# levayz/diffusion_finetuning

Measured on AMD Instinct MI355X. Metric: images/s SD1.5 LoRA rank-4 512^2 train step, higher is better.
Workload: dtype f16; 1 GPU; SD1.5 UNet-only LoRA rank=4, batch=4/GPU, 512^2 (64x64x4 latents), f16 storage/compute, fp32 accumulate + fp32 master LoRA, full train step (fwd+bwd+clip+AdamW); global_batch=4, parallelism=dp1, lora_params=1246464, overflow=False, hipgraph=True, conv_autotune=True, rccl_ranks=1

## Files before the change

### diffusion_finetuning_amd/_native.py

```python
import ctypes
import os
import threading

import torch

_LIB_PATH = os.environ.get("DFA_LIB_PATH") or os.path.join(os.path.dirname(os.path.abspath(__file__)), "lib", "liblora_hip.so")
_lib = None
_lock = threading.Lock()

ABI_VERSION = 9
PROF_KINDS = 18

_DTYPE_CODE = {torch.float32: 0, torch.float16: 1, torch.bfloat16: 2}

_vp, _i64, _i32, _f32 = ctypes.c_void_p, ctypes.c_int64, ctypes.c_int, ctypes.c_float


class GradProblem(ctypes.Structure):
    _fields_ = [
        ("S", _vp), ("P", _vp), ("out", _vp * 4),
        ("s_stride", _i64), ("p_stride", _i64), ("part_stride", _i64), ("M", _i64),
        ("C", _i32), ("r", _i32), ("rg", _i32), ("out_kn", _i32), ("n_blocks", _i32),
        ("scale", _f32),
    ]
# ... 67 lines not shown
                                       ctypes.c_uint64, ctypes.c_uint64, _i32, _i32, _vp]),
    "ddpm_posterior_sample": (_i32, [_vp, _i32, _vp, _vp, _i32, _i64, _f32, _vp]),
    "ddpm_noise_prologue_offset": (_i32, [_vp, _vp, _vp, _vp, _vp, _vp, _vp, _i32, _i64, _i32, ctypes.c_uint64, ctypes.c_uint64,
                                          _i32, _i32, _i64, _f32, _vp, _vp]),
    "ddpm_posterior_prologue_offset": (_i32, [_vp, _i32, _vp, _vp, _vp, _vp, _vp, _vp, _vp, _vp, _i32, _i64, _i32, _f32,
                                              ctypes.c_uint64, ctypes.c_uint64, _i32, _i32, _i64, _f32, _vp, _vp]),
    "ddpm_sample_init": (_i32, [_vp, _vp, _vp, _vp, _vp, _i32, _i64, _i32, _i32, ctypes.c_uint64, _i32, _vp]),
    "ddpm_sample_step": (_i32, [_vp, _vp, _vp, _vp, _vp, _vp, _vp, _vp, _i32, _i64, _i32, _i32, _f32, _i32, _vp]),
    "ddpm_sample_advance": (_i32, [_vp, _i32, _vp]),
    "ddpm_sample_multistep": (_i32, [_vp, _vp, _vp, _vp, _vp, _vp, _vp, _vp, _vp, _vp, _i32, _i64, _i32, _i32, _f32, _i32, _vp]),
    "ddpm_sample_init_from": (_i32, [_vp, _vp, _vp, _vp, _vp, _vp, _vp, _i32, _i64, _i32, _i32, _f32, _f32, _i32, ctypes.c_uint64,
                                     _i32, _vp]),
    "ddpm_sample_step_keep": (_i32, [_vp] * 11 + [_i32, _i64, _i64, _i32, _i32, _f32, _i32, _vp]),
    "ddpm_sample_multistep_keep": (_i32, [_vp] * 13 + [_i32, _i64, _i64, _i32, _i32, _f32, _i32, _vp]),
    "ddpm_sample_init_shared": (_i32, [_vp, _vp, _vp, _vp, _vp, _i32, _i64, _i32, _i32, ctypes.c_uint64, _i32, _vp]),
    "ddpm_sample_step_shared": (_i32, [_vp, _vp, _vp, _vp, _vp, _vp, _vp, _vp, _i32, _i64, _i32, _i32, _f32, _i32, _vp]),
    "ddpm_sample_init_from_shared": (_i32, [_vp, _vp, _vp, _vp, _vp, _vp, _vp, _i32, _i64, _i32, _i32, _f32, _f32, _i32,
                                            ctypes.c_uint64, _i32, _vp]),
    "ddpm_sample_step_keep_shared": (_i32, [_vp] * 11 + [_i32, _i64, _i64, _i32, _i32, _f32, _i32, _vp]),
    "ddpm_sample_multistep_keep_shared": (_i32, [_vp] * 13 + [_i32, _i64, _i64, _i32, _i32, _f32, _i32, _vp]),
    "ddpm_sample_sigma_init": (_i32, [_vp] * 7 + [_i32, _i64, _i32, _i32, _f32, _f32, _f32, _i32, _i32, ctypes.c_uint64, _i32, _vp]),
    "ddpm_sample_sigma": (_i32, [_vp] * 14 + [_i32, _i64, _i64, _i32, _i32, _i32, _f32, _i32, _vp]),
    "ddpm_cfg_rescale": (_i32, [_vp, _vp, _i32, _i64, _f32, _f32, _i32, _vp]),
    "embed_rows_fwd": (_i32, [_vp, _vp, _vp, _i64, _i32, _i64, _i32, _vp]),
    "embed_rows_bwd": (_i32, [_vp, _vp, _vp, _vp, _i64, _i32, _i64, _i32, _i32, _vp]),
    "lora_adamw_rows": (_i32, [_vp, _vp, _vp, _vp, _vp, _i64, _i32, _vp, _f32, _f32, _f32, _f32, _f32, _f32, _f32, _i32, _vp]),
    "ti_rows_grad": (_i32, [_vp, _vp, _i64, _i32, _vp, _i32, _vp, _i32, _i32, _vp]),
    "ti_rows_adamw_decay": (_i32, [_vp, _i64, _i32, _vp, _i32, _vp, _vp, _vp, _f32, _f32, _f32, _f32, _f32, _f32, _i32, _f32, _f32,
                                   _vp]),
    "geglu_linear_bwd": (_i32, [_vp, _vp, _vp, _vp, _vp, _i64, _i32, _i32, _i32, _vp]),
    "geglu_gate_fwd": (_i32, [_vp, _vp, _i64, _i32, _i32, _vp]),
    "geglu_gate_bwd": (_i32, [_vp, _vp, _vp, _i64, _i32, _i32, _vp]),
    "attn_split_heads": (_i32, [_vp, _vp, _i32, _i32, _i32, _i32, _i32, _i32, _vp]),
    "attn_merge_heads": (_i32, [_vp, _vp, _i32, _i32, _i32, _i32, _i32, _i32, _vp]),
    "attn_merge_heads_strided": (_i32, [_vp, _vp, _i32, _i32, _i32, _i32, _i32, _i64, _i64, _i64, _i32, _vp]),
    "group_norm_act_workspace_bytes": (_i64, [_i32, _i32, _i32, _i32, _i32, _i32]),
    "group_norm_act_plan": (_i32, [_i32, _i32, _i32, _i32, _i32, _i32]),
    "group_norm_act_fwd": (_i32, [_vp] * 8 + [_i32, _i32, _i32, _i32, _f32, _i32, _i32, _i32, _vp]),
    "group_norm_act_bwd": (_i32, [_vp] * 10 + [_i32, _i32, _i32, _i32, _i32, _i32, _i32, _vp]),
    "group_norm_act_bwd_res": (_i32, [_vp] * 11 + [_i32, _i32, _i32, _i32, _i32, _i32, _vp]),
    "residual_bias_add_supported": (_i32, [_i32, _i32, _i32, _i32]),
    "residual_bias_add": (_i32, [_vp] * 5 + [_i32, _i32, _i32, _i32, _vp]),
    "tokens_nchw_supported": (_i32, [_i32, _i32, _i32, _i32]),
    "tokens_to_nchw_add": (_i32, [_vp] * 3 + [_i32, _i32, _i32, _i32, _vp]),
    "nchw_to_tokens": (_i32, [_vp] * 2 + [_i32, _i32, _i32, _i32, _vp]),
    "time_proj_supported": (_i32, [_i32, _i32, _i32]),
    "time_proj_all": (_i32, [_vp] * 6 + [_i32, _i32, _i32, _i32, _vp]),
    "conv3x3_small_supported": (_i32, [_i32, _i32, _i32, _i32, _i32, _i32]),
    "conv3x3_small_workspace_bytes": (_i64, [_i32, _i32, _i32, _i32, _i32, _i32]),
    "conv3x3_small_plan": (_i32, [_i64, _i32, _i32, _i32]),
    "conv3x3_small_plan_channels": (_i32, [_i32, _i32, _i32]),
    "conv3x3_small_pack": (_i32, [_vp, _vp, _i32, _i32, _i32, _i32, _vp]),
    "conv3x3_small": (_i32, [_vp] * 5 + [_i64, _i32, _i32, _i32, _i32, _i32, _i32, _vp]),
    "conv3x3_large_supported": (_i32, [_i32, _i32, _i32, _i32, _i32, _i32]),
    "conv3x3_large_workspace_bytes": (_i64, [_i32, _i32, _i32, _i32, _i32, _i32]),
    "conv3x3_large_plan": (_i32, [_i64, _i32, _i32, _i32]),
    "conv3x3_large_plan_channels": (_i32, [_i32, _i32, _i32]),
    "conv3x3_large": (_i32, [_vp] * 5 + [_i64, _i32, _i32, _i32, _i32, _i32, _i32, _vp]),
    "conv3x3_large_tile_choice": (_i32, [_i32, _i32, _i32, _i32, _i32, _i32]),
    "conv3x3_large_tile": (_i32, [_vp] * 5 + [_i64, _i32, _i32, _i32, _i32, _i32, _i32, _i32, _vp]),
    "add_layer_norm_max_channels": (_i32, []),
    "add_layer_norm_fwd": (_i32, [_vp] * 8 + [_i64, _i32, _f32, _i32, _vp]),
    "add_layer_norm_bwd": (_i32, [_vp] * 7 + [_i64, _i32, _i32, _vp]),
    "attn_ctx_supported": (_i32, [_i32, _i32, _i32, _i32, _i32, _i32]),
    "attn_ctx_fwd": (_i32, [_vp, _vp, _vp, _vp, _i32, _i32, _i32, _i32, _i32, _f32, _i32, _vp]),
    "attn_ctx_bwd_workspace_bytes": (_i64, [_i32, _i32, _i32, _i32, _i32]),
    "attn_ctx_fwd_strided": (_i32, [_vp, _vp, _vp, _vp, _i64, _i32, _i32, _i32, _i32, _i32, _f32, _i32, _vp]),
    "attn_ctx_bwd_strided": (_i32, [_vp] * 8 + [_i64, _i64, _i32, _i32, _i32, _i32, _i32, _f32, _i32, _vp]),
    "attn_flash_fwd_strided": (_i32, [_vp, _vp, _vp, _vp, _vp, _i64, _i32, _i32, _i32, _i32, _i32, _f32, _i32, _vp]),
    "attn_flash_bwd_strided": (_i32, [_vp] * 10 + [_i64, _i64, _i32, _i32, _i32, _i32, _i32, _f32, _i32, _vp]),
    "attn_ctx_bwd": (_i32, [_vp, _vp, _vp, _vp, _vp, _vp, _vp, _vp, _i32, _i32, _i32, _i32, _i32, _f32, _i32, _vp]),
    "attn_causal_supported": (_i32, [_i32, _i32, _i32, _i32, _i32]),
    "attn_causal_fwd_strided": (_i32, [_vp, _vp, _vp, _vp, _i64, _i32, _i32, _i32, _i32, _f32, _i32, _vp]),
    "attn_causal_bwd_workspace_bytes": (_i64, [_i32, _i32, _i32, _i32]),
    "attn_causal_bwd_strided": (_i32, [_vp] * 8 + [_i64, _i64, _i32, _i32, _i32, _i32, _f32, _i32, _vp]),
    "attn_flash_supported": (_i32, [_i32, _i32, _i32, _i32, _i32, _i32]),
    "attn_flash_fwd": (_i32, [_vp, _vp, _vp, _vp, _vp, _i32, _i32, _i32, _i32, _i32, _f32, _i32, _vp]),
    "attn_flash_bwd_workspace_bytes": (_i64, [_i32, _i32, _i32]),
    "attn_flash_bwd": (_i32, [_vp] * 10 + [_i32, _i32, _i32, _i32, _i32, _f32, _i32, _vp]),
    "attn_f32_supported": (_i32, [_i32, _i32, _i32, _i32, _i32]),
    "attn_f32_fwd": (_i32, [_vp, _vp, _vp, _vp, _vp, _i32, _i32, _i32, _i32, _i32, _f32, _vp]),
    "attn_f32_bwd_workspace_bytes": (_i64, [_i32, _i32, _i32]),
    "attn_f32_bwd": (_i32, [_vp] * 10 + [_i32, _i32, _i32, _i32, _i32, _f32, _vp]),
    "lora_distill_workspace_bytes": (_i64, [_i64, _i64]),
    "lora_distill_start": (_i32, [_vp, _i32, _i64, _i32, _i64, _vp, _vp]),
    "lora_distill_diff": (_i32, [_vp, _i32, _i64, _i32, _i32, _vp, _vp]),
    "lora_distill_rayleigh_ritz": (_i32, [_vp, _i32, _i32, _i32, ctypes.c_double, _i32, _vp, _vp]),
    "lora_distill_finalize": (_i32, [_vp, _i32, _i32, _f32, _i32, _vp, _vp, _vp]),
    "lora_quantile_clamp": (_i32, [_vp, _i64, _f32, _vp, _vp]),
    "lora_distill_wide_width": (_i32, [_i32]),
    "lora_distill_wide_workspace_bytes": (_i64, [_i64, _i64, _i32]),
    "lora_distill_wide_start": (_i32, [_vp, _i32, _i64, _i32, _i64, _vp, _vp]),
    "lora_distill_wide_diff": (_i32, [_vp, _i32, _i64, _i32, _i32, _i32, _vp, _vp]),
    "lora_distill_wide_rayleigh_ritz": (_i32, [_vp, _i32, _i32, _i32, ctypes.c_double, _i32, _vp, _vp]),
    "lora_distill_wide_finalize": (_i32, [_vp, _i32, _i32, _f32, _i32, _vp, _vp, _vp]),
    "lora_prof_enable": (_i32, [_i32]),
    "lora_prof_collect": (_i32, [ctypes.POINTER(ProfTotals)]),
    "lora_prof_null_mode": (_i32, [_i32]),
    "lora_prof_kernel_name": (ctypes.c_char_p, [_i32]),
}


def library_path() -> str:
    return _LIB_PATH


def lib():
# ... 1210 lines not shown
def time_proj_supported(N: int, E: int, dtype) -> bool:
    return dtype in (torch.float16, torch.bfloat16) and bool(lib().time_proj_supported(N, E, dtype_code(dtype)))


def time_proj_all(temb, weights, biases, extra_biases):
    _require_device(temb, *weights)
    N, E = temb.shape
    L = len(weights)
    widths = [w.shape[0] for w in weights]
    out = torch.empty(N * sum(widths), dtype=temb.dtype, device=temb.device)
    ptrs = lambda ts: (_vp * L)(*[None if t is None else t.data_ptr() for t in ts])
    _check(lib().time_proj_all(_ptr(temb), ptrs(weights), ptrs(biases), ptrs(extra_biases), (_i32 * L)(*widths), _ptr(out), L, N, E,
                               dtype_code(temb.dtype), _stream(temb)), "time_proj_all")
    outs, off = [], 0
    for c in widths:
        outs.append(out[off:off + N * c].view(N, c))
        off += N * c
    return outs


def conv3x3_small_supported(N: int, Cin: int, Cout: int, H: int, W: int, dtype) -> bool:
    return dtype in (torch.float16, torch.bfloat16) and bool(lib().conv3x3_small_supported(N, Cin, Cout, H, W, dtype_code(dtype)))


def conv3x3_small_plan(pixels: int, Cin: int, Cout: int, dtype) -> bool:
    return dtype in (torch.float16, torch.bfloat16) and bool(lib().conv3x3_small_plan(int(pixels), Cin, Cout, dtype_code(dtype)))


def conv3x3_small_plan_channels(Cin: int, Cout: int, dtype) -> bool:
    return dtype in (torch.float16, torch.bfloat16) and bool(lib().conv3x3_small_plan_channels(Cin, Cout, dtype_code(dtype)))


def conv3x3_small_pack(weight, backward: bool):
    _require_device(weight)
    Cout, Cin = weight.shape[:2]
    packed = torch.empty(weight.numel(), dtype=weight.dtype, device=weight.device)
    _check(lib().conv3x3_small_pack(_ptr(weight), _ptr(packed), Cin, Cout, int(backward), dtype_code(weight.dtype),
                                    _stream(weight)), "conv3x3_small_pack")
    return packed


def conv3x3_small(x, pack, bias, Cout: int):
    _require_device(x, pack, bias)
    N, Cin, H, W = x.shape
    code = dtype_code(x.dtype)
    nbytes = int(lib().conv3x3_small_workspace_bytes(N, Cin, Cout, H, W, code))
    ws = torch.empty(max(nbytes, 16) // 4, dtype=torch.float32, device=x.device)
    y = torch.empty((N, Cout, H, W), dtype=x.dtype, device=x.device)
    _check(lib().conv3x3_small(_ptr(x), _ptr(pack), _ptr(bias), _ptr(y), _ptr(ws), nbytes, N, Cin, Cout, H, W, code, _stream(x)),
           "conv3x3_small")
    return y


def conv3x3_large_supported(N: int, Cin: int, Cout: int, H: int, W: int, dtype) -> bool:
    return dtype in (torch.float16, torch.bfloat16) and bool(lib().conv3x3_large_supported(N, Cin, Cout, H, W, dtype_code(dtype)))


def conv3x3_large_plan(pixels: int, Cin: int, Cout: int, dtype) -> bool:
    return dtype in (torch.float16, torch.bfloat16) and bool(lib().conv3x3_large_plan(int(pixels), Cin, Cout, dtype_code(dtype)))


def conv3x3_large_plan_channels(Cin: int, Cout: int, dtype) -> bool:
    return dtype in (torch.float16, torch.bfloat16) and bool(lib().conv3x3_large_plan_channels(Cin, Cout, dtype_code(dtype)))


def conv3x3_large(x, pack, bias, Cout: int):
    _require_device(x, pack, bias)
    N, Cin, H, W = x.shape
    y = torch.empty((N, Cout, H, W), dtype=x.dtype, device=x.device)
    _check(lib().conv3x3_large(_ptr(x), _ptr(pack), _ptr(bias), _ptr(y), None, 0, N, Cin, Cout, H, W, dtype_code(x.dtype),
                               _stream(x)), "conv3x3_large")
    return y


def conv3x3_large_tile_choice(N: int, Cin: int, Cout: int, H: int, W: int, dtype) -> int:
    if dtype not in (torch.float16, torch.bfloat16):
        return -1
    return int(lib().conv3x3_large_tile_choice(N, Cin, Cout, H, W, dtype_code(dtype)))


def conv3x3_large_tile(x, pack, bias, Cout: int, tile: int):
    _require_device(x, pack, bias)
    N, Cin, H, W = x.shape
    y = torch.empty((N, Cout, H, W), dtype=x.dtype, device=x.device)
    _check(lib().conv3x3_large_tile(_ptr(x), _ptr(pack), _ptr(bias), _ptr(y), None, 0, N, Cin, Cout, H, W, dtype_code(x.dtype),
                                    int(tile), _stream(x)), "conv3x3_large_tile")
    return y


def tokens_nchw_supported(N: int, C: int, HW: int, dtype) -> bool:
    return dtype in (torch.float16, torch.bfloat16) and bool(lib().tokens_nchw_supported(N, C, HW, dtype_code(dtype)))


def tokens_to_nchw_add(tok, res, shape):
    _require_device(tok, res)
    N, C, H, W = shape
    out = torch.empty(shape, dtype=tok.dtype, device=tok.device)
    _check(lib().tokens_to_nchw_add(_ptr(tok), _ptr(res), _ptr(out), N, C, H * W, dtype_code(tok.dtype), _stream(tok)),
           "tokens_to_nchw_add")
    return out


def nchw_to_tokens(x):
    _require_device(x)
    N, C, H, W = x.shape
    tok = torch.empty((N, H * W, C), dtype=x.dtype, device=x.device)
# ... 278 lines not shown
```

### diffusion_finetuning_amd/csrc/conv_small.hip

```cpp
#include "conv_common.h"

namespace {

constexpr int kNT = 128;

template <typename T, int MT, int PER>
__global__ __launch_bounds__(kThreads) void conv_small_kernel(const T* __restrict__ x, const T* __restrict__ wp,
                                                              float* __restrict__ part, int Cin, int Cout, int H, int W, int M,
                                                              int mtiles, int ntiles, int cps, int chunks, int Mpad) {
    using Frag = typename Mfma<T>::Frag;
    constexpr int MF = MT / 32;
    extern __shared__ __attribute__((aligned(16))) unsigned char smem[];
    const int tid = threadIdx.x, lane = tid & 63, wave = tid >> 6, wm = wave & 1, wn = wave >> 1;

    int mt, nt, sl;
    {
        const unsigned total = gridDim.x, id = blockIdx.x;
        const unsigned q = total >> 3, rem = total & 7, xcd = id & 7, slot = id >> 3;
        const unsigned n = (xcd < rem ? xcd * (q + 1) : rem * (q + 1) + (xcd - rem) * q) + slot;
        mt = (int)(n % (unsigned)mtiles);
        const unsigned rest = n / (unsigned)mtiles;
        nt = (int)(rest % (unsigned)ntiles);
        sl = (int)(rest / (unsigned)ntiles);
    }
    const int c_begin = sl * cps, c_end = min(c_begin + cps, chunks);
    const int HW = H * W, W2 = W + 2, PP = (H + 2) * W2;
    const int m0 = mt * MT;
    const int q0 = padded_pos(m0, H, W);
    const int P = tile_positions(m0, MT, M, H, W);
    const int qlo = q0 - (W2 + 1);
    const float inv_pp = 1.f / (float)PP, inv_w2 = 1.f / (float)W2;

    int xoff[PER];
    bool in_tile[PER];
#pragma unroll
    for (int s = 0; s < PER; ++s) {
        const int p = tid + s * kThreads;
        const int q = qlo + p, img = fast_div(q, PP, inv_pp), r = q - img * PP, hp = fast_div(r, W2, inv_w2), wq = r - hp * W2;
        in_tile[s] = p < P;
        const bool inside = in_tile[s] && hp >= 1 && hp <= H && wq >= 1 && wq <= W;
        xoff[s] = inside ? img * Cin * HW + (hp - 1) * W + (wq - 1) : -1;
    }
    T raw[PER][32];
    auto load_stage = [&](int cc) {
        const T* base = x + (size_t)cc * kChunk * HW;
#pragma unroll
        for (int s = 0; s < PER; ++s) {
            const int o = xoff[s] >= 0 ? xoff[s] : 0;
#pragma unroll
            for (int c = 0; c < 32; ++c) raw[s][c] = base[o + c * HW];
        }
    };

    int lpos[MF];
    const float inv_hw = 1.f / (float)HW, inv_w = 1.f / (float)W;
#pragma unroll
    for (int f = 0; f < MF; ++f) {
        const int m = min(m0 + wm * (MT / 2) + f * 16 + (lane & 15), M - 1);
        const int img = fast_div(m, HW, inv_hw), r = m - img * HW, h = fast_div(r, W, inv_w);
        lpos[f] = (img * PP + (h + 1) * W2 + (r - h * W) + 1 - q0) * kPitch + (lane >> 4) * 16;
    }
    const int KO = Cout >> 4;
    int wofs[4];
#pragma unroll
    for (int g = 0; g < 4; ++g) wofs[g] = min(nt * (kNT / 16) + wn * 4 + g, KO - 1) * 512 + lane * 8;
    const size_t tap_stride = (size_t)KO * 512;
    const int L_end = c_end * 9;
    Frag wf[9][4];
    auto load_w = [&](int slot, int L) {
        const T* src = wp + (size_t)min(L, L_end - 1) * tap_stride;
#pragma unroll
        for (int g = 0; g < 4; ++g) wf[slot][g] = *reinterpret_cast<const Frag*>(src + wofs[g]);
    };

    f32x4 acc[MF][4];
#pragma unroll
    for (int f = 0; f < MF; ++f)
#pragma unroll
        for (int g = 0; g < 4; ++g) acc[f][g] = f32x4{0.f, 0.f, 0.f, 0.f};

    load_stage(c_begin);
#pragma unroll
    for (int t = 0; t < 9; ++t) load_w(t, c_begin * 9 + t);
    for (int cc = c_begin; cc < c_end; ++cc) {
        __syncthreads();
#pragma unroll
        for (int s = 0; s < PER; ++s)
            if (in_tile[s]) {
#pragma unroll
                for (int c8 = 0; c8 < 4; ++c8) {
                    Frag v;
#pragma unroll
                    for (int j = 0; j < 8; ++j) v[j] = xoff[s] >= 0 ? raw[s][c8 * 8 + j] : static_cast<T>(0.f);
                    *reinterpret_cast<Frag*>(smem + (tid + s * kThreads) * kPitch + c8 * 16) = v;
                }
            }
        __syncthreads();
        load_stage(min(cc + 1, c_end - 1));
        __builtin_amdgcn_sched_barrier(0);
        Frag xf[2][MF];
#pragma unroll
        for (int f = 0; f < MF; ++f) xf[0][f] = *reinterpret_cast<const Frag*>(smem + lpos[f]);
#pragma unroll
        for (int t = 0; t < 9; ++t) {
            if (t + 1 < 9) {
                const int sh = (((t + 1) / 3) * W2 + ((t + 1) % 3)) * kPitch;
#pragma unroll
                for (int f = 0; f < MF; ++f) xf[(t + 1) & 1][f] = *reinterpret_cast<const Frag*>(smem + lpos[f] + sh);
            }
#pragma unroll
            for (int f = 0; f < MF; ++f)
#pragma unroll
                for (int g = 0; g < 4; ++g) acc[f][g] = Mfma<T>::run(xf[t & 1][f], wf[t][g], acc[f][g]);
            load_w(t, cc * 9 + t + 9);
            __builtin_amdgcn_sched_barrier(0);
        }
    }

#pragma unroll
    for (int g = 0; g < 4; ++g) {
        const int k = nt * kNT + wn * 64 + g * 16 + (lane & 15);
        if (k < Cout) {
            float* dst = part + ((size_t)sl * Cout + k) * Mpad + m0 + wm * (MT / 2) + (lane >> 4) * 4;
#pragma unroll
            for (int f = 0; f < MF; ++f) *reinterpret_cast<f32x4*>(dst + f * 16) = acc[f][g];
        }
    }
}

template <typename T, int V>
__global__ __launch_bounds__(256) void conv_small_reduce_kernel(const float* __restrict__ part, const T* __restrict__ bias,
                                                                T* __restrict__ y, int Cout, int HW, int M, int Mpad, int S) {
    const int idx = blockIdx.x * 256 + threadIdx.x, MV = M / V;
    if (idx >= Cout * MV) return;
    const int k = idx / MV, m = (idx - k * MV) * V;
    const float* src = part + (size_t)k * Mpad + m;
    const size_t stride = (size_t)Cout * Mpad;
    float v[V];
    if constexpr (V == 4) {
        f32x4 a = *reinterpret_cast<const f32x4*>(src);
        int s = 1;
        for (; s + 3 < S; s += 4) {
            const f32x4 b0 = *reinterpret_cast<const f32x4*>(src + s * stride), b1 = *reinterpret_cast<const f32x4*>(src + (s + 1) * stride),
                        b2 = *reinterpret_cast<const f32x4*>(src + (s + 2) * stride), b3 = *reinterpret_cast<const f32x4*>(src + (s + 3) * stride);
            a += b0, a += b1, a += b2, a += b3;
        }
        for (; s < S; ++s) a += *reinterpret_cast<const f32x4*>(src + s * stride);
#pragma unroll
        for (int i = 0; i < 4; ++i) v[i] = a[i];
    } else {
        v[0] = src[0];
        for (int s = 1; s < S; ++s) v[0] += src[s * stride];
    }
    const float b = bias ? to_f32(bias[k]) : 0.f;
    const int n = m / HW, p = m - n * HW;
    T* dst = y + ((size_t)n * Cout + k) * HW + p;
    if constexpr (V == 4) {
        struct alignas(8) Out4 { T v[4]; } o;
#pragma unroll
        for (int i = 0; i < 4; ++i) o.v[i] = from_f32<T>(v[i] + b);
        *reinterpret_cast<Out4*>(dst) = o;
    } else {
        dst[0] = from_f32<T>(v[0] + b);
    }
}

template <typename T>
__global__ __launch_bounds__(256) void conv_small_pack_kernel(const T* __restrict__ w, T* __restrict__ out, int Cin, int Cout,
                                                              int backward) {
    const int64_t total = (int64_t)Cin * Cout * 9, o = (int64_t)blockIdx.x * 256 + threadIdx.x;
    if (o >= total) return;
    const int Co = backward ? Cin : Cout, KO = Co >> 4;
    const int j = (int)(o & 7), l = (int)((o >> 3) & 63);
    const int64_t rest = o >> 9;
    const int ko = (int)(rest % KO);
    const int64_t rest2 = rest / KO;
    const int t = (int)(rest2 % 9), cc = (int)(rest2 / 9);
    const int ci = cc * 32 + (l >> 4) * 8 + j, co = ko * 16 + (l & 15);
    const int64_t src = backward ? ((int64_t)ci * Cin + co) * 9 + (8 - t) : ((int64_t)co * Cin + ci) * 9 + t;
    out[o] = w[src];
}

struct Geo {
    int MT = 0, per = 0, mtiles = 0, ntiles = 0, chunks = 0, cps = 0, S = 0, Pcap = 0, Mpad = 0, M = 0;
    int64_t ws_bytes = 0;
    bool ok = false;
};

Geo conv_geo(int N, int Cin, int Cout, int H, int W) {
    Geo g;
    if (!conv_shape_in_range(N, Cin, Cout, H, W)) return g;
    const int M = N * H * W;
    const int mts[2] = {128, 64}, per[2] = {1, 3};
    for (int v = 0; v < 2 && !g.ok; ++v) {
        const int MT = mts[v], mtiles = (M + MT - 1) / MT;
        int pmax = 0;
        for (int t = 0; t < mtiles; ++t) {
            const int p = tile_positions(t * MT, MT, M, H, W);
            pmax = p > pmax ? p : pmax;
        }
        if (pmax > per[v] * kThreads) continue;
        g.MT = MT, g.per = per[v], g.mtiles = mtiles, g.Pcap = pmax, g.ok = true;
    }
    if (!g.ok) return g;
    g.M = M;
    g.Mpad = g.mtiles * g.MT;
    g.ntiles = (Cout + kNT - 1) / kNT;
    g.chunks = Cin / kChunk;
    const int tiles = g.mtiles * g.ntiles, want = kCUs / tiles > 1 ? kCUs / tiles : 1;
    int cps = (g.chunks + want - 1) / want;
    if (g.chunks >= 4 && cps < 2) cps = 2;
    g.cps = cps;
    g.S = (g.chunks + cps - 1) / cps;
    g.ws_bytes = (int64_t)g.S * Cout * g.Mpad * 4;
    if ((int64_t)tiles * g.S > (1 << 20)) g.ok = false;
    return g;
}

template <typename T, int MT, int PER>
bool launch_main(const T* x, const T* wp, float* part, int Cin, int Cout, int H, int W, const Geo& g, hipStream_t s) {
    const int lds = g.Pcap * kPitch;
    auto kern = conv_small_kernel<T, MT, PER>;
    if (lds > 48 * 1024 &&
        hipFuncSetAttribute(reinterpret_cast<const void*>(kern), hipFuncAttributeMaxDynamicSharedMemorySize, lds) != hipSuccess)
        return false;
    hipLaunchKernelGGL(kern, dim3(g.mtiles * g.ntiles * g.S), dim3(kThreads), lds, s, x, wp, part, Cin, Cout, H, W, g.M, g.mtiles,
                       g.ntiles, g.cps, g.chunks, g.Mpad);
    return true;
}

template <typename T>
int run_conv(const void* x_, const void* wp_, const void* bias_, void* y_, void* ws, int Cin, int Cout, int H, int W, const Geo& g,
             hipStream_t s) {
    const T *x = static_cast<const T*>(x_), *wp = static_cast<const T*>(wp_), *bias = static_cast<const T*>(bias_);
    float* part = static_cast<float*>(ws);
    const bool ok = g.MT == 128 ? launch_main<T, 128, 1>(x, wp, part, Cin, Cout, H, W, g, s)
                                : launch_main<T, 64, 3>(x, wp, part, Cin, Cout, H, W, g, s);
    if (!ok) return LORA_E_LAUNCH;
    if ((H * W) % 4 == 0) {
        const int total = Cout * (g.M / 4);
        hipLaunchKernelGGL((conv_small_reduce_kernel<T, 4>), dim3((total + 255) / 256), dim3(256), 0, s, part, bias, static_cast<T*>(y_),
                           Cout, H * W, g.M, g.Mpad, g.S);
    } else {
        const int total = Cout * g.M;
        hipLaunchKernelGGL((conv_small_reduce_kernel<T, 1>), dim3((total + 255) / 256), dim3(256), 0, s, part, bias, static_cast<T*>(y_),
                           Cout, H * W, g.M, g.Mpad, g.S);
    }
    LORA_LAUNCH_CHECK();
    return LORA_OK;
}

}

extern "C" int conv3x3_small_supported(int N, int C_in, int C_out, int H, int W, int dtype) {
    return (dtype == LORA_F16 || dtype == LORA_BF16) && conv_geo(N, C_in, C_out, H, W).ok ? 1 : 0;
}

extern "C" int64_t conv3x3_small_workspace_bytes(int N, int C_in, int C_out, int H, int W, int dtype) {
    if (!conv3x3_small_supported(N, C_in, C_out, H, W, dtype)) return 0;
    return conv_geo(N, C_in, C_out, H, W).ws_bytes;
}

namespace {
bool plan_channels(int C_in, int C_out, int64_t pixels ) {
    if (C_in != 1280 && C_out != 1280) return false;
    const int other = C_in == 1280 ? C_out : C_in;
    const bool at256 = other == 1280 || other == 2560;
    const bool at1024 = other == 640 || other == 1280 || other == 1920 || other == 2560;
    return pixels == 256 ? at256 : pixels == 1024 ? at1024 : pixels == 0 ? (at256 || at1024) : false;
}
}

extern "C" int conv3x3_small_plan(int64_t pixels, int C_in, int C_out, int dtype) {
    if (dtype != LORA_F16 && dtype != LORA_BF16) return 0;
    return pixels >= 1 && plan_channels(C_in, C_out, pixels) ? 1 : 0;
}

extern "C" int conv3x3_small_plan_channels(int C_in, int C_out, int dtype) {
    if (dtype != LORA_F16 && dtype != LORA_BF16) return 0;
    return plan_channels(C_in, C_out, 0) ? 1 : 0;
}

extern "C" int conv3x3_small_pack(const void* w, void* packed, int C_in, int C_out, int backward, int dtype, void* stream) {
    if (!w || !packed || C_in < 1 || C_out < 1 || (backward != 0 && backward != 1)) return LORA_E_BADARG;
    if (dtype != LORA_F16 && dtype != LORA_BF16) return dtype == LORA_F32 ? LORA_E_UNSUPPORTED : LORA_E_BADARG;
    if (C_in % 32 || C_out % 32) return LORA_E_UNSUPPORTED;
    if (!aligned16(packed)) return LORA_E_ALIGN;
    const int64_t total = (int64_t)C_in * C_out * 9;
    if (total >= (1ll << 31)) return LORA_E_UNSUPPORTED;
    hipStream_t s = static_cast<hipStream_t>(stream);
    const dim3 grid((unsigned)((total + 255) / 256));
    if (dtype == LORA_F16)
        hipLaunchKernelGGL(conv_small_pack_kernel<half_t>, grid, dim3(256), 0, s, static_cast<const half_t*>(w),
                           static_cast<half_t*>(packed), C_in, C_out, backward);
    else
        hipLaunchKernelGGL(conv_small_pack_kernel<bf16_t>, grid, dim3(256), 0, s, static_cast<const bf16_t*>(w),
                           static_cast<bf16_t*>(packed), C_in, C_out, backward);
    LORA_LAUNCH_CHECK();
    return LORA_OK;
}

extern "C" int conv3x3_small(const void* x, const void* wpack, const void* bias, void* y, void* workspace, int64_t workspace_bytes,
                             int N, int C_in, int C_out, int H, int W, int dtype, void* stream) {
    if (!x || !wpack || !y || !workspace || N < 1 || C_in < 1 || C_out < 1 || H < 1 || W < 1) return LORA_E_BADARG;
    if (dtype != LORA_F16 && dtype != LORA_BF16) return dtype == LORA_F32 ? LORA_E_UNSUPPORTED : LORA_E_BADARG;
    const Geo g = conv_geo(N, C_in, C_out, H, W);
    if (!g.ok) return LORA_E_UNSUPPORTED;
    if (workspace_bytes < g.ws_bytes) return LORA_E_BADARG;
    if (!aligned16(x) || !aligned16(wpack) || !aligned16(y) || !aligned16(workspace)) return LORA_E_ALIGN;
    hipStream_t s = static_cast<hipStream_t>(stream);
    return dtype == LORA_F16 ? run_conv<half_t>(x, wpack, bias, y, workspace, C_in, C_out, H, W, g, s)
                             : run_conv<bf16_t>(x, wpack, bias, y, workspace, C_in, C_out, H, W, g, s);
}
```

### include/lora_hip.h

```cpp
#ifndef LORA_HIP_H
#define LORA_HIP_H

#include <stdint.h>

#ifdef __cplusplus
extern "C" {
#endif

#define LORA_HIP_ABI_VERSION 9

enum lora_dtype { LORA_F32 = 0, LORA_F16 = 1, LORA_BF16 = 2 };

enum lora_status {
    LORA_OK = 0,
    LORA_E_BADARG = -1,
    LORA_E_RANK = -2,
    LORA_E_ALIGN = -3,
    LORA_E_LAUNCH = -4,
    LORA_E_UNSUPPORTED = -5
};

int lora_version(void);

const char* lora_status_string(int status);
// ... 196 lines not shown
                                      void* stream);

int ddpm_sample_sigma_init(float* x, void* model_in, float* t_model, int* cursor, const float* timesteps,
                           const float* init , float* eps_out , int B, int64_t per_row, int I,
                           int start, float k, float nn, float c_in, int cfg, int shared, uint64_t seed, int dtype, void* stream);
int ddpm_sample_sigma(float* x, float* xs, float* hist, const void* model_out, void* model_in, float* t_model, const int* cursor,
                      const float* timesteps, const float* coef, const int* plan, float* z_out ,
                      const float* mask , const float* init , const float* keep_coef ,
                      int B, int64_t per_row, int64_t hw, int I, int cfg, int shared, float guidance_scale, int dtype,
                      void* stream);

int ddpm_cfg_rescale(void* model_out, float* k_out , int B, int64_t per_row, float guidance_scale, float rescale,
                     int dtype, void* stream);

int geglu_gate_fwd(const void* y, void* out, int64_t M, int C, int dtype, void* stream);
int geglu_gate_bwd(const void* y, const void* dout, void* dy, int64_t M, int C, int dtype, void* stream);
int attn_split_heads(const void* src, void* dst, int B, int N, int H, int d, int D, int dtype, void* stream);
int attn_merge_heads(const void* src, void* dst, int B, int N, int H, int d, int D, int dtype, void* stream);
int attn_merge_heads_strided(const void* src, void* dst, int B, int N, int H, int d, int D, int64_t sB, int64_t sH,
                             int64_t sN, int dtype, void* stream);

int64_t group_norm_act_workspace_bytes(int N, int C, int HW, int groups, int channels_last, int want_da);
int group_norm_act_plan(int N, int C, int HW, int groups, int channels_last, int backward);
int group_norm_act_fwd(const void* x, const void* addend , const void* gamma, const void* beta, void* y,
                       float* mean, float* rstd, void* workspace, int N, int C, int HW, int groups, float eps, int act,
                       int channels_last, int dtype, void* stream);
int group_norm_act_bwd(const void* dy, const void* x, const void* addend , const void* gamma, const void* beta,
                       const float* mean, const float* rstd, void* dx, void* da , void* workspace, int N, int C,
                       int HW, int groups, int act, int channels_last, int dtype, void* stream);
int group_norm_act_bwd_res(const void* dy, const void* dh , const void* x, const void* addend ,
                           const void* gamma, const void* beta, const float* mean, const float* rstd, void* dx,
                           void* da , void* workspace, int N, int C, int HW, int groups, int act, int dtype,
                           void* stream);

int residual_bias_add_supported(int N, int C, int HW, int dtype);
int residual_bias_add(const void* h, const void* res, const void* b1, const void* b2 , void* out, int N, int C,
                      int HW, int dtype, void* stream);
int tokens_nchw_supported(int N, int C, int HW, int dtype);
int tokens_to_nchw_add(const void* tok, const void* res , void* out, int N, int C, int HW, int dtype,
                       void* stream);
int nchw_to_tokens(const void* x, void* tok, int N, int C, int HW, int dtype, void* stream);

int time_proj_supported(int N, int E, int dtype);
int time_proj_all(const void* t, const void* const* W, const void* const* b , const void* const* cb ,
                  const int* C, void* out, int L, int N, int E, int dtype, void* stream);

int conv3x3_small_supported(int N, int C_in, int C_out, int H, int W, int dtype);
int64_t conv3x3_small_workspace_bytes(int N, int C_in, int C_out, int H, int W, int dtype);
int conv3x3_small_plan(int64_t pixels, int C_in, int C_out, int dtype);
int conv3x3_small_plan_channels(int C_in, int C_out, int dtype);
int conv3x3_small_pack(const void* w, void* packed, int C_in, int C_out, int backward, int dtype, void* stream);
int conv3x3_small(const void* x, const void* wpack, const void* bias , void* y, void* workspace,
                  int64_t workspace_bytes, int N, int C_in, int C_out, int H, int W, int dtype, void* stream);

int conv3x3_large_supported(int N, int C_in, int C_out, int H, int W, int dtype);
int64_t conv3x3_large_workspace_bytes(int N, int C_in, int C_out, int H, int W, int dtype);
int conv3x3_large_plan(int64_t pixels, int C_in, int C_out, int dtype);
int conv3x3_large_plan_channels(int C_in, int C_out, int dtype);
int conv3x3_large(const void* x, const void* wpack, const void* bias , void* y, void* workspace ,
                  int64_t workspace_bytes, int N, int C_in, int C_out, int H, int W, int dtype, void* stream);
int conv3x3_large_tile_choice(int N, int C_in, int C_out, int H, int W, int dtype);
int conv3x3_large_tile(const void* x, const void* wpack, const void* bias , void* y, void* workspace ,
                       int64_t workspace_bytes, int N, int C_in, int C_out, int H, int W, int dtype, int tile, void* stream);

int add_layer_norm_max_channels(void);
int add_layer_norm_fwd(const void* x, const void* delta , const void* gamma, const void* beta,
                       void* h , void* y, float* mean, float* rstd, int64_t M, int C, float eps,
                       int dtype, void* stream);
int add_layer_norm_bwd(const void* dy, const void* dh , const void* h, const void* gamma, const float* mean,
                       const float* rstd, void* dx, int64_t M, int C, int dtype, void* stream);

int embed_rows_fwd(const float* table, const int64_t* ids, void* out, int64_t n, int D, int64_t V, int out_dtype, void* stream);
int embed_rows_bwd(const void* dE, const int64_t* ids, float* grad_table, unsigned char* active , int64_t n,
                   int D, int64_t V, int dtype, int accumulate, void* stream);
int lora_adamw_rows(float* param, const float* grad, float* exp_avg, float* exp_avg_sq, const unsigned char* active, int64_t V,
                    int D, const float* norm_in, float grad_mul, float max_norm, float lr, float beta1, float beta2, float eps,
                    float weight_decay, int step, void* stream);

#define LORA_TI_MAX_ROWS 64
int ti_rows_grad(const void* dE, const int64_t* ids, int64_t n, int D, const int64_t* slot_ids, int P, float* grad, int dtype,
                 int accumulate, void* stream);
int ti_rows_adamw_decay(float* table, int64_t V, int D, const int64_t* slot_ids, int P, const float* grad, float* exp_avg,
                        float* exp_avg_sq, float grad_mul, float lr, float beta1, float beta2, float eps, float weight_decay,
                        int step, float decay_lambda, float target_norm, void* stream);

int attn_ctx_supported(int B, int Tq, int Tk, int H, int d, int dtype);
int attn_ctx_fwd_strided(const void* Q, const void* K, const void* V, void* O, int64_t ldk, int B, int Tq, int Tk,
                         int H, int d, float scale, int dtype, void* stream);
int attn_ctx_bwd_strided(const void* Q, const void* K, const void* V, const void* dO, void* dQ, void* dK, void* dV,
                         void* workspace, int64_t ldk, int64_t ld_dk, int B, int Tq, int Tk, int H, int d,
                         float scale, int dtype, void* stream);
int attn_ctx_fwd(const void* Q, const void* K, const void* V, void* O, int B, int Tq, int Tk, int H, int d,
                 float scale, int dtype, void* stream);
int64_t attn_ctx_bwd_workspace_bytes(int B, int Tq, int Tk, int H, int d);
int attn_ctx_bwd(const void* Q, const void* K, const void* V, const void* dO, void* dQ, void* dK, void* dV,
                 void* workspace, int B, int Tq, int Tk, int H, int d, float scale, int dtype, void* stream);

int attn_causal_supported(int B, int T, int H, int d, int dtype);
int attn_causal_fwd_strided(const void* Q, const void* K, const void* V, void* O, int64_t ldq, int B, int T, int H, int d,
                            float scale, int dtype, void* stream);
int64_t attn_causal_bwd_workspace_bytes(int B, int T, int H, int d);
int attn_causal_bwd_strided(const void* Q, const void* K, const void* V, const void* dO, void* dQ, void* dK, void* dV,
                            void* workspace, int64_t ldq, int64_t ld_dq, int B, int T, int H, int d, float scale,
                            int dtype, void* stream);

int attn_flash_supported(int B, int Tq, int Tk, int H, int d, int dtype);
// ... 58 lines not shown
```

Measured before the change: 210.1 images/s.

## Add row-vectorized, double-buffered LDS staging form to small 3x3 conv

Adds a 'rows' form to the small-spatial conv3x3 kernel. It loads input rows as 16-byte vectors and interleaves channel pairs into LDS instead of doing scalar per-position gathers. It also double-buffers the LDS stage, so the write of the next chunk follows the MFMA loop and only one barrier is needed per chunk. The default path picks the rows form for N=4 at 8x8 and 16x16 with swept channel counts, and it caches the LDS-attribute call. The cost is twice the LDS footprint, which can lower occupancy, and a one-time zero-fill of LDS.

```diff
diff --git a/diffusion_finetuning_amd/_native.py b/diffusion_finetuning_amd/_native.py
--- a/diffusion_finetuning_amd/_native.py
+++ b/diffusion_finetuning_amd/_native.py
@@ -143,7 +143,9 @@
     "conv3x3_small_plan_channels": (_i32, [_i32, _i32, _i32]),
     "conv3x3_small_pack": (_i32, [_vp, _vp, _i32, _i32, _i32, _i32, _vp]),
     "conv3x3_small": (_i32, [_vp] * 5 + [_i64, _i32, _i32, _i32, _i32, _i32, _i32, _vp]),
-    "conv3x3_large_supported": (_i32, [_i32, _i32, _i32, _i32, _i32, _i32]),
+    "conv3x3_small_form_choice": (_i32, [_i32, _i32, _i32, _i32, _i32, _i32]),
+    "conv3x3_small_form": (_i32, [_vp] * 5 + [_i64, _i32, _i32, _i32, _i32, _i32, _i32, _i32, _vp]),
+    "conv3x3_large_supported":(_i32, [_i32, _i32, _i32, _i32, _i32, _i32]),
     "conv3x3_large_workspace_bytes": (_i64, [_i32, _i32, _i32, _i32, _i32, _i32]),
     "conv3x3_large_plan": (_i32, [_i64, _i32, _i32, _i32]),
     "conv3x3_large_plan_channels": (_i32, [_i32, _i32, _i32]),
@@ -1460,6 +1462,24 @@
     return y
 
 
+def conv3x3_small_form_choice(N: int, Cin: int, Cout: int, H: int, W: int, dtype) -> int:
+    if dtype not in (torch.float16, torch.bfloat16):
+        return -1
+    return int(lib().conv3x3_small_form_choice(N, Cin, Cout, H, W, dtype_code(dtype)))
+
+
+def conv3x3_small_form(x, pack, bias, Cout: int, form: int):
+    _require_device(x, pack, bias)
+    N, Cin, H, W = x.shape
+    code = dtype_code(x.dtype)
+    nbytes = int(lib().conv3x3_small_workspace_bytes(N, Cin, Cout, H, W, code))
+    ws = torch.empty(max(nbytes, 16) // 4, dtype=torch.float32, device=x.device)
+    y = torch.empty((N, Cout, H, W), dtype=x.dtype, device=x.device)
+    _check(lib().conv3x3_small_form(_ptr(x), _ptr(pack), _ptr(bias), _ptr(y), _ptr(ws), nbytes, N, Cin, Cout, H, W, code, int(form),
+                                    _stream(x)), "conv3x3_small_form")
+    return y
+
+
 def conv3x3_large_supported(N: int, Cin: int, Cout: int, H: int, W: int, dtype) -> bool:
     return dtype in (torch.float16, torch.bfloat16) and bool(lib().conv3x3_large_supported(N, Cin, Cout, H, W, dtype_code(dtype)))
 
diff --git a/diffusion_finetuning_amd/csrc/conv_small.hip b/diffusion_finetuning_amd/csrc/conv_small.hip
--- a/diffusion_finetuning_amd/csrc/conv_small.hip
+++ b/diffusion_finetuning_amd/csrc/conv_small.hip
@@ -1,15 +1,22 @@
+#include <atomic>
+
 #include "conv_common.h"
 
 namespace {
 
 constexpr int kNT = 128;
 
-template <typename T, int MT, int PER>
+__device__ __forceinline__ void lds_barrier() { asm volatile("s_waitcnt lgkmcnt(0)\n\ts_barrier" ::: "memory"); }
+
+template <typename T, int MT, int PER, int RU>
 __global__ __launch_bounds__(kThreads) void conv_small_kernel(const T* __restrict__ x, const T* __restrict__ wp,
                                                               float* __restrict__ part, int Cin, int Cout, int H, int W, int M,
                                                               int mtiles, int ntiles, int cps, int chunks, int Mpad) {
     using Frag = typename Mfma<T>::Frag;
     constexpr int MF = MT / 32;
+    constexpr bool ROWS = RU > 0;
+    constexpr int kBuf = PER * kThreads * kPitch;
+    constexpr int NU = ROWS ? RU : 1;
     extern __shared__ __attribute__((aligned(16))) unsigned char smem[];
     const int tid = threadIdx.x, lane = tid & 63, wave = tid >> 6, wm = wave & 1, wn = wave >> 1;
 
@@ -31,26 +38,85 @@
     const int qlo = q0 - (W2 + 1);
     const float inv_pp = 1.f / (float)PP, inv_w2 = 1.f / (float)W2;
 
-    int xoff[PER];
-    bool in_tile[PER];
-#pragma unroll
-    for (int s = 0; s < PER; ++s) {
-        const int p = tid + s * kThreads;
-        const int q = qlo + p, img = fast_div(q, PP, inv_pp), r = q - img * PP, hp = fast_div(r, W2, inv_w2), wq = r - hp * W2;
-        in_tile[s] = p < P;
-        const bool inside = in_tile[s] && hp >= 1 && hp <= H && wq >= 1 && wq <= W;
-        xoff[s] = inside ? img * Cin * HW + (hp - 1) * W + (wq - 1) : -1;
-    }
-    T raw[PER][32];
+    int xoff[ROWS ? NU : PER];
+    int aoff[NU];
+    if constexpr (ROWS) {
+        const int S = W >> 3, lb = (S & 1) ^ 1, S2 = S >> lb;
+        const int img0 = m0 / HW, h0 = (m0 - img0 * HW) / W;
+        const bool whole = MT % HW == 0;
+        const int images = min(MT / HW, (M - m0) / HW);
+#pragma unroll
+        for (int s = 0; s < RU; ++s) {
+            const int i = tid + s * kThreads, cp = (i >> lb) & 15, rest = i >> (4 + lb);
+            int k = rest / S2;
+            const int seg = (i & lb) + ((rest - k * S2) << lb);
+            const bool unit = whole ? k < images * H : (k < MT / W + 2 && h0 - 1 + k >= 0 && h0 - 1 + k < H);
+            if (!unit) k = whole ? 0 : 1;
+            const int im = whole ? k / H : 0, hr = whole ? k - im * H : h0 - 1 + k;
+            const int j = whole ? im * (H + 2) + hr + 1 : k;
+            xoff[s] = ((img0 + im) * Cin + 2 * cp) * HW + hr * W + 8 * seg;
+            aoff[s] = (j * W2 + 1 + 8 * seg) * kPitch + cp * 4;
+        }
+    } else {
+#pragma unroll
+        for (int s = 0; s < PER; ++s) {
+            const int p = tid + s * kThreads;
+            const int q = qlo + p, img = fast_div(q, PP, inv_pp), r = q - img * PP, hp = fast_div(r, W2, inv_w2), wq = r - hp * W2;
+            const bool inside = p < P && hp >= 1 && hp <= H && wq >= 1 && wq <= W;
+            xoff[s] = inside ? img * Cin * HW + (hp - 1) * W + (wq - 1) : -1;
+        }
+    }
+    T raw[ROWS ? 1 : PER][32];
+    uint4 rawr[NU][2];
     auto load_stage = [&](int cc) {
         const T* base = x + (size_t)cc * kChunk * HW;
-#pragma unroll
-        for (int s = 0; s < PER; ++s) {
-            const int o = xoff[s] >= 0 ? xoff[s] : 0;
-#pragma unroll
-            for (int c = 0; c < 32; ++c) raw[s][c] = base[o + c * HW];
+        if constexpr (ROWS) {
+#pragma unroll
+            for (int s = 0; s < RU; ++s) {
+                rawr[s][0] = *reinterpret_cast<const uint4*>(base + xoff[s]);
+                rawr[s][1] = *reinterpret_cast<const uint4*>(base + xoff[s] + HW);
+            }
+        } else {
+#pragma unroll
+            for (int s = 0; s < PER; ++s) {
+                const int o = xoff[s] >= 0 ? xoff[s] : 0;
+#pragma unroll
+                for (int c = 0; c < 32; ++c) raw[s][c] = base[o + c * HW];
+            }
         }
     };
+    auto write_stage = [&](int buf) {
+        unsigned char* dstb = smem + buf * kBuf;
+        if constexpr (ROWS) {
+#pragma unroll
+            for (int s = 0; s < RU; ++s) {
+                unsigned char* dst = dstb + aoff[s];
+                const unsigned a[4] = {rawr[s][0].x, rawr[s][0].y, rawr[s][0].z, rawr[s][0].w};
+                const unsigned b[4] = {rawr[s][1].x, rawr[s][1].y, rawr[s][1].z, rawr[s][1].w};
+#pragma unroll
+                for (int k = 0; k < 4; ++k) {
+                    *reinterpret_cast<unsigned*>(dst + (2 * k) * kPitch) = (a[k] & 0xffffu) | (b[k] << 16);
+                    *reinterpret_cast<unsigned*>(dst + (2 * k + 1) * kPitch) = (a[k] >> 16) | (b[k] & 0xffff0000u);
+                }
+            }
+        } else {
+#pragma unroll
+            for (int s = 0; s < PER; ++s)
+#pragma unroll
+                for (int c8 = 0; c8 < 4; ++c8) {
+                    Frag v;
+#pragma unroll
+                    for (int j = 0; j < 8; ++j) v[j] = xoff[s] >= 0 ? raw[s][c8 * 8 + j] : static_cast<T>(0.f);
+                    *reinterpret_cast<Frag*>(dstb + (tid + s * kThreads) * kPitch + c8 * 16) = v;
+                }
+        }
+    };
+    if constexpr (ROWS) {
+#pragma unroll
+        for (int i = 0; i < 2 * kBuf / (16 * kThreads); ++i)
+            *reinterpret_cast<uint4*>(smem + (i * kThreads + tid) * 16) = uint4{0u, 0u, 0u, 0u};
+        lds_barrier();
+    }
 
     int lpos[MF];
     const float inv_hw = 1.f / (float)HW, inv_w = 1.f / (float)W;
@@ -80,33 +146,25 @@
         for (int g = 0; g < 4; ++g) acc[f][g] = f32x4{0.f, 0.f, 0.f, 0.f};
 
     load_stage(c_begin);
+    __builtin_amdgcn_sched_barrier(0);
 #pragma unroll
     for (int t = 0; t < 9; ++t) load_w(t, c_begin * 9 + t);
+    __builtin_amdgcn_sched_barrier(0);
+    write_stage(c_begin & 1);
+    lds_barrier();
     for (int cc = c_begin; cc < c_end; ++cc) {
-        __syncthreads();
-#pragma unroll
-        for (int s = 0; s < PER; ++s)
-            if (in_tile[s]) {
-#pragma unroll
-                for (int c8 = 0; c8 < 4; ++c8) {
-                    Frag v;
-#pragma unroll
-                    for (int j = 0; j < 8; ++j) v[j] = xoff[s] >= 0 ? raw[s][c8 * 8 + j] : static_cast<T>(0.f);
-                    *reinterpret_cast<Frag*>(smem + (tid + s * kThreads) * kPitch + c8 * 16) = v;
-                }
-            }
-        __syncthreads();
+        const unsigned char* ab = smem + (cc & 1) * kBuf;
         load_stage(min(cc + 1, c_end - 1));
         __builtin_amdgcn_sched_barrier(0);
         Frag xf[2][MF];
 #pragma unroll
-        for (int f = 0; f < MF; ++f) xf[0][f] = *reinterpret_cast<const Frag*>(smem + lpos[f]);
+        for (int f = 0; f < MF; ++f) xf[0][f] = *reinterpret_cast<const Frag*>(ab + lpos[f]);
 #pragma unroll
         for (int t = 0; t < 9; ++t) {
             if (t + 1 < 9) {
                 const int sh = (((t + 1) / 3) * W2 + ((t + 1) % 3)) * kPitch;
 #pragma unroll
-                for (int f = 0; f < MF; ++f) xf[(t + 1) & 1][f] = *reinterpret_cast<const Frag*>(smem + lpos[f] + sh);
+                for (int f = 0; f < MF; ++f) xf[(t + 1) & 1][f] = *reinterpret_cast<const Frag*>(ab + lpos[f] + sh);
             }
 #pragma unroll
             for (int f = 0; f < MF; ++f)
@@ -115,6 +173,8 @@
             load_w(t, cc * 9 + t + 9);
             __builtin_amdgcn_sched_barrier(0);
         }
+        write_stage((cc + 1) & 1);
+        lds_barrier();
     }
 
 #pragma unroll
@@ -217,13 +277,25 @@
     return g;
 }
 
-template <typename T, int MT, int PER>
+constexpr int kFormPosition = 0, kFormRows = 1;
+
+int rows_units(const Geo& g, int H, int W) {
+    if (!g.ok || g.MT != 128 || W % 8 || 128 % W) return 0;
+    const int HW = H * W;
+    if (128 % HW == 0) return 1;
+    return HW % 128 == 0 && 256 + 4 * W <= 2 * kThreads ? 2 : 0;
+}
+
+template <typename T, int MT, int PER, int RU>
 bool launch_main(const T* x, const T* wp, float* part, int Cin, int Cout, int H, int W, const Geo& g, hipStream_t s) {
-    const int lds = g.Pcap * kPitch;
-    auto kern = conv_small_kernel<T, MT, PER>;
-    if (lds > 48 * 1024 &&
-        hipFuncSetAttribute(reinterpret_cast<const void*>(kern), hipFuncAttributeMaxDynamicSharedMemorySize, lds) != hipSuccess)
-        return false;
+    constexpr int lds = 2 * PER * kThreads * kPitch;
+    auto kern = conv_small_kernel<T, MT, PER, RU>;
+    static std::atomic<bool> raised{false};
+    if (lds > 48 * 1024 && !raised.load(std::memory_order_relaxed)) {
+        if (hipFuncSetAttribute(reinterpret_cast<const void*>(kern), hipFuncAttributeMaxDynamicSharedMemorySize, lds) != hipSuccess)
+            return false;
+        raised.store(true, std::memory_order_relaxed);
+    }
     hipLaunchKernelGGL(kern, dim3(g.mtiles * g.ntiles * g.S), dim3(kThreads), lds, s, x, wp, part, Cin, Cout, H, W, g.M, g.mtiles,
                        g.ntiles, g.cps, g.chunks, g.Mpad);
     return true;
@@ -231,11 +303,13 @@
 
 template <typename T>
 int run_conv(const void* x_, const void* wp_, const void* bias_, void* y_, void* ws, int Cin, int Cout, int H, int W, const Geo& g,
-             hipStream_t s) {
+             int ru, hipStream_t s) {
     const T *x = static_cast<const T*>(x_), *wp = static_cast<const T*>(wp_), *bias = static_cast<const T*>(bias_);
     float* part = static_cast<float*>(ws);
-    const bool ok = g.MT == 128 ? launch_main<T, 128, 1>(x, wp, part, Cin, Cout, H, W, g, s)
-                                : launch_main<T, 64, 3>(x, wp, part, Cin, Cout, H, W, g, s);
+    const bool ok = ru == 1     ? launch_main<T, 128, 1, 1>(x, wp, part, Cin, Cout, H, W, g, s)
+                    : ru == 2   ? launch_main<T, 128, 1, 2>(x, wp, part, Cin, Cout, H, W, g, s)
+                    : g.MT == 128 ? launch_main<T, 128, 1, 0>(x, wp, part, Cin, Cout, H, W, g, s)
+                                  : launch_main<T, 64, 3, 0>(x, wp, part, Cin, Cout, H, W, g, s);
     if (!ok) return LORA_E_LAUNCH;
     if ((H * W) % 4 == 0) {
         const int total = Cout * (g.M / 4);
@@ -268,6 +342,27 @@
     const bool at256 = other == 1280 || other == 2560;
     const bool at1024 = other == 640 || other == 1280 || other == 1920 || other == 2560;
     return pixels == 256 ? at256 : pixels == 1024 ? at1024 : pixels == 0 ? (at256 || at1024) : false;
+}
+
+int measured_form(const Geo& g, int N, int Cin, int Cout, int H, int W) {
+    const bool swept = N == 4 && H == W && (H == 8 || H == 16) && plan_channels(Cin, Cout, (int64_t)N * H * W);
+    return swept && rows_units(g, H, W) ? kFormRows : kFormPosition;
+}
+
+int small_call(const void* x, const void* wpack, const void* bias, void* y, void* workspace, int64_t workspace_bytes, int N, int C_in,
+               int C_out, int H, int W, int dtype, int form, void* stream) {
+    if (!x || !wpack || !y || !workspace || N < 1 || C_in < 1 || C_out < 1 || H < 1 || W < 1) return LORA_E_BADARG;
+    if (dtype != LORA_F16 && dtype != LORA_BF16) return dtype == LORA_F32 ? LORA_E_UNSUPPORTED : LORA_E_BADARG;
+    const Geo g = conv_geo(N, C_in, C_out, H, W);
+    if (!g.ok) return LORA_E_UNSUPPORTED;
+    if (form < 0) form = measured_form(g, N, C_in, C_out, H, W);
+    const int ru = form == kFormRows ? rows_units(g, H, W) : 0;
+    if (form == kFormRows && !ru) return LORA_E_UNSUPPORTED;
+    if (workspace_bytes < g.ws_bytes) return LORA_E_BADARG;
+    if (!aligned16(x) || !aligned16(wpack) || !aligned16(y) || !aligned16(workspace)) return LORA_E_ALIGN;
+    hipStream_t s = static_cast<hipStream_t>(stream);
+    return dtype == LORA_F16 ? run_conv<half_t>(x, wpack, bias, y, workspace, C_in, C_out, H, W, g, ru, s)
+                             : run_conv<bf16_t>(x, wpack, bias, y, workspace, C_in, C_out, H, W, g, ru, s);
 }
 }
 
@@ -302,13 +397,18 @@
 
 extern "C" int conv3x3_small(const void* x, const void* wpack, const void* bias, void* y, void* workspace, int64_t workspace_bytes,
                              int N, int C_in, int C_out, int H, int W, int dtype, void* stream) {
-    if (!x || !wpack || !y || !workspace || N < 1 || C_in < 1 || C_out < 1 || H < 1 || W < 1) return LORA_E_BADARG;
-    if (dtype != LORA_F16 && dtype != LORA_BF16) return dtype == LORA_F32 ? LORA_E_UNSUPPORTED : LORA_E_BADARG;
+    return small_call(x, wpack, bias, y, workspace, workspace_bytes, N, C_in, C_out, H, W, dtype, -1, stream);
+}
+
+extern "C" int conv3x3_small_form_choice(int N, int C_in, int C_out, int H, int W, int dtype) {
+    if (dtype != LORA_F16 && dtype != LORA_BF16) return -1;
     const Geo g = conv_geo(N, C_in, C_out, H, W);
-    if (!g.ok) return LORA_E_UNSUPPORTED;
-    if (workspace_bytes < g.ws_bytes) return LORA_E_BADARG;
-    if (!aligned16(x) || !aligned16(wpack) || !aligned16(y) || !aligned16(workspace)) return LORA_E_ALIGN;
-    hipStream_t s = static_cast<hipStream_t>(stream);
-    return dtype == LORA_F16 ? run_conv<half_t>(x, wpack, bias, y, workspace, C_in, C_out, H, W, g, s)
-                             : run_conv<bf16_t>(x, wpack, bias, y, workspace, C_in, C_out, H, W, g, s);
-}
+    return g.ok ? measured_form(g, N, C_in, C_out, H, W) : -1;
+}
+
+extern "C" int conv3x3_small_form(const void* x, const void* wpack, const void* bias, void* y, void* workspace,
+                                  int64_t workspace_bytes, int N, int C_in, int C_out, int H, int W, int dtype, int form,
+                                  void* stream) {
+    if (form != kFormPosition && form != kFormRows) return LORA_E_BADARG;
+    return small_call(x, wpack, bias, y, workspace, workspace_bytes, N, C_in, C_out, H, W, dtype, form, stream);
+}
diff --git a/include/lora_hip.h b/include/lora_hip.h
--- a/include/lora_hip.h
+++ b/include/lora_hip.h
@@ -272,6 +272,9 @@
 int conv3x3_small_pack(const void* w, void* packed, int C_in, int C_out, int backward, int dtype, void* stream);
 int conv3x3_small(const void* x, const void* wpack, const void* bias , void* y, void* workspace,
                   int64_t workspace_bytes, int N, int C_in, int C_out, int H, int W, int dtype, void* stream);
+int conv3x3_small_form_choice(int N, int C_in, int C_out, int H, int W, int dtype);
+int conv3x3_small_form(const void* x, const void* wpack, const void* bias , void* y, void* workspace,
+                       int64_t workspace_bytes, int N, int C_in, int C_out, int H, int W, int dtype, int form, void* stream);
 
 int conv3x3_large_supported(int N, int C_in, int C_out, int H, int W, int dtype);
 int64_t conv3x3_large_workspace_bytes(int N, int C_in, int C_out, int H, int W, int dtype);
```

Measured after the change: 214.4 images/s (median of 6 runs). +2.0%, better.
